# xiph/LPCNet

Hardware: AMD Instinct MI355X
Metric: 16 kHz samples/sec & concurrent real-time streams, 1/2/4/8 MI355X (higher is better)
Workload: dtype f32; 1 GPU; 2048 concurrent streams (each with its own feature file) per GPU x 25 frames (4000 samples) per step, fp32 weights, register-resident block-sparse GRU-A, bit-exact (PARITY) arithmetic; eight streams per CU as two groups of four half a step apart (BASELINE config 2's 1024 streams fill half of these stream slots: `also.config2_1024_streams`); arithmetic=parity, gru_a_blocks=1382, gru_a_densities=0.05,0.05,0.2 (benchmark model), gru_a_items_per_lane=30, streams_per_gpu=2048, streams_per_workgroup=8

## Files before the change

### lpcnet_amd/csrc/sample_kernel_x2.hip.h

```cpp
#pragma once
#include "sample_kernel.hip.h"
#include "tree_stages.h"

namespace lpcn {

#define LPCN_X2_LW 4
#define LPCN_X2_TW 0
#define LPCN_X2_S2W 7
#define LPCN_X2_S2_LEAD 2
#define LPCN_X2_HG 10

struct LdsX2 {
    static constexpr int S = 4;
    static constexpr int HA_STRIDE = 16 * S;
    static constexpr int g_hA    = 0;
    static constexpr int g_hT    = g_hA + 96 * HA_STRIDE + 24 * 16;
    static constexpr int g_prec  = g_hT + NA * S * 4;
    static constexpr int g_hB    = g_prec + NA * S * 4;
    static constexpr int g_idx   = g_hB + S * NB * 4;
    static constexpr int g_thr   = g_idx + S * 16;
    static constexpr int g_mask  = g_thr + S * 32;
    static constexpr int g_pfx   = g_mask + S * 4;
    static constexpr int g_lead  = g_mask + S * 64;
    static constexpr int g_flag  = g_lead + S * 32;
    static constexpr int g_condb = g_flag + 16;
    static constexpr int g_lpc   = g_condb + S * RB * 4;
    static constexpr int g_pcm   = g_lpc + S * 64;
    static constexpr int G_SZ    = g_pcm + S * 320;
    static constexpr int pre_ur  = 2 * G_SZ;
    static constexpr int inh     = pre_ur + 2 * NA * S * 4;
    static constexpr int abias   = inh + NA * S * 4;
    static constexpr int tansig  = abias + 2 * RA * 4;
    static constexpr int ulaw    = tansig + 816;
    static constexpr int logit   = ulaw + 1024;
    static constexpr int brec    = logit + 1024;
    static constexpr int bbias   = brec + NB * RB * 4;
    static constexpr int bstart  = bbias + 2 * RB * 4;
    static constexpr int bw      = bstart + 32;
    static constexpr int total(int nb_b) { return bw + (nb_b + 8) * 128; }
    __host__ __device__ static constexpr int ha_off(int p) { return p * HA_STRIDE + (p >> 2) * 16; }
};

typedef float tree_f4 __attribute__((ext_vector_type(4)));
struct TreeRow { tree_f4 w[NB / 4]; float bias, factor; };
__device__ __forceinline__ TreeRow tree_row_load_node(const LPCN_GLOBAL float *fc_w, const LPCN_GLOBAL float *fc_b, const LPCN_GLOBAL float *fc_f, const int node, const int chan)
{
    const auto *wp = (const LPCN_GLOBAL tree_f4 *)(fc_w + (node * 2 + chan) * NB);
    TreeRow r;
#pragma unroll
    for (int j = 0; j < NB / 4; ++j) r.w[j] = wp[j];
    r.bias = fc_b[chan * 256 + node];
    r.factor = fc_f[chan * 256 + node];
    return r;
}
template <int STAGE>
__device__ __forceinline__ TreeRow tree_row_load(const LPCN_GLOBAL float *fc_w, const LPCN_GLOBAL float *fc_b, const LPCN_GLOBAL float *fc_f, const int lane, const int prefix)
{
    return tree_row_load_node(fc_w, fc_b, fc_f, lpcn_tree_node(STAGE, lpcn_tree_lane_local(STAGE, lane), prefix), lane & 1);
}
__device__ __forceinline__ TreeRow tree_row_load_packed(const LPCN_GLOBAL float *fc_w, const LPCN_GLOBAL float *fc_b, const LPCN_GLOBAL float *fc_f, const int lane, const int prefix)
{
    return tree_row_load_node(fc_w, fc_b, fc_f, lpcn_tree_packed_node(lane, prefix), lane & 1);
}
__device__ __forceinline__ unsigned long long tree_node_ballot(const TreeRow &r, const float *h_s, const float *thr, const float *tansig)
{
    const float4 *hp = (const float4 *)h_s;
    float sum = r.bias;
#pragma unroll
    for (int j = 0; j < NB / 4; ++j) {
        const float4 hv = hp[j];
        const tree_f4 wv = r.w[j];
        sum = sum + wv[0] * hv.x;
        sum = sum + wv[1] * hv.y;
        sum = sum + wv[2] * hv.z;
        sum = sum + wv[3] * hv.w;
    }
    const float v = r.factor * lpcn_tanh(sum, tansig);
    const float vo = __builtin_bit_cast(float, __builtin_amdgcn_mov_dpp(__builtin_bit_cast(int, v), 0xB1, 0xf, 0xf, true));
    const float lg = v + vo;
    return __ballot(*thr < lg);
}
template <int STAGE>
__device__ __forceinline__ int tree_stage_walk(const TreeRow &r, const float *h_s, const float *thr_s, const float *tansig, const int lane)
{
    const unsigned long long m = tree_node_ballot(r, h_s, thr_s + lpcn_tree_level(STAGE, lpcn_tree_lane_local(STAGE, lane)), tansig) & lpcn_tree_stage_mask(STAGE);
    return lpcn_tree_stage_walk(m, STAGE == 0 ? LPCN_TREE_TOP : LPCN_TREE_LEVELS - LPCN_TREE_TOP);
}

template <int NW>
__global__ __launch_bounds__(LPCN_WG_THREADS, 2) void sample_kernel_x2(const LpcnSampleArgs *__restrict__ Ap)
{
    using L = LdsX2;
    constexpr int S = 4;
    constexpr int LW = LPCN_X2_LW, TW = LPCN_X2_TW;
    extern __shared__ __attribute__((aligned(16))) unsigned char smem[];
    float *const sm_pre_ur = (float *)(smem + L::pre_ur);
    float *const sm_inh = (float *)(smem + L::inh);
    const float *const sm_abias = (const float *)(smem + L::abias);
    const float *const sm_tansig = (const float *)(smem + L::tansig);
    const float *const sm_ulaw = (const float *)(smem + L::ulaw);
    const float *const sm_logit = (const float *)(smem + L::logit);
    const float *const sm_brec = (const float *)(smem + L::brec);
    const float *const sm_bbias = (const float *)(smem + L::bbias);
    const int *const sm_bstart = (const int *)(smem + L::bstart);

    const int tid0 = threadIdx.x;
    const int n_streams = Ap->n_streams, n_frames = Ap->n_frames, preload = Ap->preload, frame_len = Ap->frame_len;
    const int s0 = blockIdx.x * 2 * S;
    auto stream_of = [&](int gs) __attribute__((always_inline)) { return (s0 + gs < n_streams) ? s0 + gs : n_streams - 1; };
    const int n_valid = (n_streams - s0 < 2 * S) ? n_streams - s0 : 2 * S;
    const size_t nf = (size_t)n_frames;
    auto *const states = as_global_rw(Ap->state);
    const LPCN_GLOBAL float *emb_nat_sig = as_global(Ap->emb_nat_sig), *emb_nat_pred = as_global(Ap->emb_nat_pred), *emb_nat_exc = as_global(Ap->emb_nat_exc);
    asm volatile("" : "+s"(emb_nat_sig), "+s"(emb_nat_pred), "+s"(emb_nat_exc));

    float4 w[NW];
    uint32_t offp[(NW + 1) / 2];
    int row_reg[3];
#define LPCN_ROW(k) (row_reg[k])
    {
        const int lane = tid0 & 63, wave = tid0 >> 6;
        const size_t base = (size_t)wave * NW * 64 + lane;
        const int lane_sel = (lane & 3) * 16;
        const auto *ab = as_global(Ap->a_blk);
        const auto *aw = (const LPCN_GLOBAL float *)as_global(Ap->a_w);
#pragma unroll
        for (int j = 0; j < NW; ++j) {
            const auto *v = aw + (base + (size_t)j * 64) * 4;
            w[j] = make_float4(v[0], v[1], v[2], v[3]);
        }
#pragma unroll
        for (int j = 0; j < NW; j += 2) {
            const int p0 = ab[base + (size_t)j * 64];
            const int p1 = (j + 1 < NW) ? ab[base + (size_t)(j + 1) * 64] : 0;
            offp[j >> 1] = (uint32_t)(L::ha_off(p0) + lane_sel) | ((uint32_t)(L::ha_off(p1) + lane_sel) << 16);
        }
        const auto *ar = as_global(Ap->a_row);
#pragma unroll
        for (int k = 0; k < 3; ++k) row_reg[k] = ar[(wave * 3 + k) * 64 + lane];
    }
    int b1 = __builtin_amdgcn_readfirstlane(as_global(Ap->a_bound)[(tid0 >> 6) * 4 + 1]);
    int b2 = __builtin_amdgcn_readfirstlane(as_global(Ap->a_bound)[(tid0 >> 6) * 4 + 2]);
    int b3 = __builtin_amdgcn_readfirstlane(as_global(Ap->a_bound)[(tid0 >> 6) * 4 + 3]);
    const bool allh0 = __builtin_amdgcn_readfirstlane(as_global(Ap->a_allh)[(tid0 >> 6) * 3]) != 0;
    const LPCN_GLOBAL float *fc_w_s = as_global(Ap->fc_w), *fc_b_s = as_global(Ap->fc_b), *fc_f_s = as_global(Ap->fc_f);
    asm volatile("" : "+s"(fc_w_s), "+s"(fc_b_s), "+s"(fc_f_s));
    const LPCN_GLOBAL float *cond_a_s = as_global(Ap->cond_a);
    asm volatile("" : "+s"(cond_a_s));
    const int has_slot = __builtin_amdgcn_readfirstlane((__ballot(row_reg[0] >= 0) != 0ull ? 1 : 0) | (__ballot(row_reg[1] >= 0) != 0ull ? 2 : 0) |
                                                        (__ballot(row_reg[2] >= 0) != 0ull ? 4 : 0));
    const bool has2 = (has_slot & 4) != 0;
    const int hl = __builtin_amdgcn_readfirstlane(as_global(Ap->a_head)[tid0 >> 6]);
    const bool early_wave = hl > 0;
    const bool plain_start = __builtin_amdgcn_readfirstlane(((early_wave || __ballot(row_reg[0] >= 2 * NA) == 0ull) && __ballot(row_reg[1] >= 2 * NA || row_reg[2] >= 2 * NA) == 0ull) ? 1 : 0) != 0;

    {
        const int tid = tid0;
        stage_tables<L>(smem, Ap, tid, NB * RB);
        stage_grub_weights(smem + L::bw, Ap, tid, true);
        for (int i = tid; i < 2 * S * NA; i += LPCN_WG_THREADS) {
            const int gs = i / NA, n = i % NA, g = gs >> 2, s = gs & 3;
            const float hv0 = states[stream_of(gs)].gru_a[n];
            unsigned char *gb = smem + g * L::G_SZ;
            ((float *)(gb + L::g_hT))[n * S + s] = hv0;
            *(float *)(gb + L::g_hA + L::ha_off(n >> 2) + s * 16 + (n & 3) * 4) = hv0;
        }
        for (int i = tid; i < 2 * S * NB; i += LPCN_WG_THREADS) {
            const int gs = i / NB, g = gs >> 2, s = gs & 3;
            ((float *)(smem + g * L::G_SZ + L::g_hB))[s * NB + i % NB] = states[stream_of(gs)].gru_b[i % NB];
        }
        if (tid < 2 * S) {
            const int g = tid >> 2, s = tid & 3;
            unsigned char *gb = smem + g * L::G_SZ;
            stage_leader_record({(float *)(gb + L::g_lead), (int *)(gb + L::g_idx), nullptr, nullptr}, s, &states[stream_of(tid)]);
        }
        if (tid < 2) { int *fl = (int *)(smem + tid * L::G_SZ + L::g_flag); fl[0] = 0; fl[1] = 0; }
        if (tid < 2 * S) ((int *)(smem + (tid >> 2) * L::G_SZ + L::g_pfx))[tid & 3] = 0;
    }
    __syncthreads();

    const bool is_lw = (tid0 >> 6) == LW;
    const bool is_tw_lane = tid0 >= 64 * TW && tid0 < 64 * TW + S;
#define LPCN_LROW ((tid0 & 63) >> 4)
#define LPCN_TAP (tid0 & 15)
    float histP = is_lw ? states[stream_of(S + LPCN_LROW)].last_sig[LPCN_TAP] : 0.f;
    float histQ = is_lw ? states[stream_of(LPCN_LROW)].last_sig[LPCN_TAP] : 0.f;
    bool liveP = false, liveQ = false;
    int live_maskP = 0, live_maskQ = 0;
    int seqP = 0, seqQ = 0;
    int smpP = 0, smpQ = 0, fP = 0, fQ = 0;
    float lpc_tap = 0.f, prod_old = 0.f;

    const int T = n_frames * frame_len;
#if LPCN_ENABLE_PROF
#ifndef LPCN_PROF_MASK
#define LPCN_PROF_MASK 0xFFF
#endif
    unsigned long long *const prof = Ap->prof;
    unsigned long long pt[12] = {0, 0, 0, 0, 0, 0, 0, 0, 0, 0, 0, 0}, tprev = 0;
    const bool profiling = prof != nullptr && blockIdx.x == 0;
#define LPCN_X2_PROF(slot) do { if (((LPCN_PROF_MASK >> (slot)) & 1) && profiling) { const unsigned long long now_ = __builtin_amdgcn_s_memtime(); pt[slot] += now_ - tprev; tprev = now_; } } while (0)
    if (profiling) tprev = __builtin_amdgcn_s_memtime();
#else
#define LPCN_X2_PROF(slot) do { } while (0)
#endif
    for (int h = -1; h <= 2 * T + 1; ++h) {
        const int p = h & 1, q = p ^ 1;
        unsigned char *const gp = smem + p * L::G_SZ, *const gq = smem + q * L::G_SZ;
        const bool p_active = h >= 0 && (h >> 1) < T;
        const bool p_prev = h >= 2;
        const bool q_chain = h >= 1 && ((h - 1) >> 1) < T;
        const bool q_heads = ((h + 1) >> 1) < T;
        const bool new_frame = p_active && smpP == 0;
        const bool more = p_active && smpP != 0;
        float *const hT_p = (float *)(gp + L::g_hT);
        float *const hB_q = (float *)(gq + L::g_hB);
        int *const idx_p = (int *)(gp + L::g_idx);
        float *const lpc_p = (float *)(gp + L::g_lpc);
        short *const pcm_p = (short *)(gp + L::g_pcm);
        const LeaderCells cells_p = {(float *)(gp + L::g_lead), idx_p, (float *)(gp + L::g_thr), pcm_p};
        const uint32_t flag_p = lds_addr(gp + L::g_flag);

        if (more) ++seqP;
        if (p_prev && is_lw) {
            __builtin_amdgcn_s_setprio(3);
            const int smp_done = smpP == 0 ? frame_len - 1 : smpP - 1;
            int t_ = tid0;
            LPCN_REMAT_V(t_);
            const int lrow = (t_ & 63) >> 4, tap = t_ & 15;
            float pcm, deemph;
            int exc;
            draw_sample_walked(cells_p, (const int *)(gp + L::g_mask) + lrow, sm_ulaw, lrow, tap, liveP, smp_done, preload, histP, pcm, deemph, exc);
            if (more) { open_sample<S>(cells_p, tid0, liveP, pcm, tap == 0 ? pcm * lpc_tap : prod_old, exc, false); lds_publish(flag_p, seqP); }
            __builtin_amdgcn_s_setprio(0);
            finish_sample(cells_p, lrow, tap, liveP, smp_done, preload, pcm, deemph);
        }
        if (more && is_tw_lane && liveP) { int t_ = tid0; LPCN_REMAT_V(t_); draw_thresholds(cells_p, sm_logit, t_ - 64 * TW); }

        if (new_frame) {
            int tid = tid0;
            LPCN_REMAT_V(tid);
            const bool lw_ = (tid >> 6) == LW, twl_ = tid >= 64 * TW && tid < 64 * TW + S;
            __syncthreads();
            if (fP > 0) {
                auto *out = as_global_rw(Ap->pcm);
                const size_t pstride = (size_t)Ap->pcm_stride;
                for (int i = tid; i < S * LPCN_FRAME_SIZE; i += LPCN_WG_THREADS) {
                    const int s = i / LPCN_FRAME_SIZE, k = i % LPCN_FRAME_SIZE;
                    if (S * p + s < n_valid && k < frame_len) out[(size_t)(s0 + S * p + s) * pstride + (size_t)(fP - 1) * LPCN_FRAME_SIZE + k] = pcm_p[i];
                }
            }
            __syncthreads();
            {
                const auto *cb = as_global(Ap->cond_b), *lp = as_global(Ap->lpc);
                float *const condb_p = (float *)(gp + L::g_condb);
                if (tid < S * RB) condb_p[tid] = cb[((size_t)stream_of(S * p + tid / RB) * nf + fP) * RB + tid % RB];
                if (tid >= 256 && tid < 256 + S * LPCN_LPC_ORDER) {
                    const int i = tid - 256;
                    lpc_p[i] = lp[((size_t)stream_of(S * p + i / LPCN_LPC_ORDER) * nf + fP) * LPCN_LPC_ORDER + i % LPCN_LPC_ORDER];
                }
                if (lw_ || twl_) {
                    const int lstream = stream_of(S * p + (lw_ ? (tid & 63) >> 4 : tid - 64 * TW));
                    liveP = stream_is_live(Ap, states, lstream, fP);
                }
                if (preload > 0 && tid < S) {
                    const auto *pin = as_global(Ap->pcm) + (size_t)stream_of(S * p + tid) * (size_t)Ap->pcm_stride + (size_t)fP * LPCN_FRAME_SIZE;
                    for (int i = 0; i < preload; ++i) pcm_p[tid * LPCN_FRAME_SIZE + i] = pin[i];
                }
            }
            __syncthreads();
            ++seqP;
            if (lw_) {
                open_sample<S>(cells_p, tid0, liveP, histP, histP * lpc_p[tid & 63], ((const int *)cells_p.lead)[((tid & 63) >> 4) * 8 + 2], true);
                lds_publish(flag_p, seqP);
            }
            if (twl_ && liveP) draw_thresholds(cells_p, sm_logit, tid - 64 * TW);
            __syncthreads();
            int lm = 0;
#pragma unroll
            for (int s = 0; s < S; ++s) lm |= (idx_p[S + s] ? 1 : 0) << s;
            live_maskP = __builtin_amdgcn_readfirstlane(lm);
        }

        LPCN_X2_PROF(0);
        float acc[S] = {};
        constexpr int PF = 2;
        float4 hq[PF + 1] = {};
        const unsigned char *hA_cur = gp + L::g_hA;
        auto fetch_h = [&](const int j) __attribute__((always_inline)) {
            uint32_t pk = offp[j >> 1];
            LPCN_REMAT_V(pk);
            const uint32_t off = (j & 1) ? (pk >> 16) : (pk & 0xFFFFu);
            hq[j % (PF + 1)] = *(const float4 *)(hA_cur + off);
        };
        typedef float negz_t __attribute__((ext_vector_type(4)));
        negz_t negz = {-0.f, -0.f, -0.f, -0.f};
        auto load_negz = [&]() __attribute__((always_inline)) { negz = (negz_t){-0.f, -0.f, -0.f, -0.f}; asm volatile("" : "+v"(negz)); };
        auto mac = [&](const int j) __attribute__((always_inline)) {
            typedef float f4 __attribute__((ext_vector_type(4)));
            typedef float f2 __attribute__((ext_vector_type(2)));
            const float4 hv = hq[j % (PF + 1)];
            const float hk[4] = {hv.x, hv.y, hv.z, hv.w};
            const float wk[4] = {w[j].x, w[j].y, w[j].z, w[j].w};
            f2 a01 = {acc[0], acc[1]}, a23 = {acc[2], acc[3]};
            f4 pv[4];
#pragma unroll
            for (int c = 0; c < 4; ++c) pv[c] = __builtin_amdgcn_mfma_f32_4x4x1f32(hk[c], wk[c], negz, 0, 0, 0);
            __builtin_amdgcn_sched_barrier(0);
#pragma unroll
            for (int c = 0; c < 4; ++c) {
                a01 = a01 + __builtin_shufflevector(pv[c], pv[c], 0, 1);
                a23 = a23 + __builtin_shufflevector(pv[c], pv[c], 2, 3);
            }
            acc[0] = a01[0]; acc[1] = a01[1]; acc[2] = a23[0]; acc[3] = a23[1];
        };
        auto pre_cell = [&](const int r, unsigned char *gb) __attribute__((always_inline)) -> float * {
            return (float *)(r < 2 * NA ? smem + L::pre_ur + r * (S * 4) : gb + L::g_prec + (r - 2 * NA) * (S * 4));
        };

        const int wave = __builtin_amdgcn_readfirstlane(tid0 >> 6);

        constexpr int J0 = NW - LPCN_EARLY_MAX < 0 ? 0 : NW - LPCN_EARLY_MAX;
        constexpr int JM = J0 + LPCN_X2_HG < NW ? J0 + LPCN_X2_HG : NW;
        const bool do_heads = early_wave && q_heads;
        int e0 = NW - hl;
        LPCN_REMAT_S(e0);
        auto head_step = [&](auto self, auto jc, auto jend_c) __attribute__((always_inline)) -> void {
            constexpr int j = decltype(jc)::value, je = decltype(jend_c)::value;
            if constexpr (j < je) {
                if constexpr (j + PF < NW) fetch_h(j + PF);
                if (j >= e0) { asm volatile(""); mac(j); }
                self(self, std::integral_constant<int, j + 1>{}, jend_c);
            }
        };
        const uint32_t p0cnt_p = flag_p + 4;
        constexpr int CW = LPCN_X2_CHAIN_WAVES, P0W = LPCN_X2_P0_FIRST, NP0 = LPCN_WAVES - P0W;
        static_assert(NP0 * 64 * 3 == 2 * NA && CW == S, "three rounds of the row waves' lanes cover GRU-A's update / reset rows");
        const bool p0_wave = p_active && wave >= P0W;
        uint32_t o_sig[S] = {}, o_pred[S] = {}, o_exc[S] = {}, o_cond[S] = {};
        constexpr int P0PERM = 0x3102;
        int i0 = 0;
        float ld[3][4 * S] = {};
        auto p0_open = [&]() __attribute__((always_inline)) {
            int gi[S];
            {
                typedef int i4 __attribute__((ext_vector_type(4)));
                i4 v;
                int f;
                const uint32_t idx_a = lds_addr(idx_p);
                do {
                    asm volatile("ds_read_b32 %0, %2\n\tds_read_b128 %1, %3\n\ts_waitcnt lgkmcnt(0)" : "=&v"(f), "=&v"(v) : "v"(flag_p), "v"(idx_a) : "memory");
                    f = __builtin_amdgcn_readfirstlane(f);
                } while (f != seqP);
#pragma unroll
                for (int s = 0; s < S; ++s) gi[s] = __builtin_amdgcn_readfirstlane(v[s]);
            }
#pragma unroll
            for (int s = 0; s < S; ++s) {
                o_sig[s] = (uint32_t)(gi[s] & 0xFF) * (uint32_t)(RA * 4);
                o_pred[s] = (uint32_t)((gi[s] >> 8) & 0xFF) * (uint32_t)(RA * 4);
                o_exc[s] = ((uint32_t)(gi[s] >> 16) & 0xFFu) * (uint32_t)(RA * 4);
                o_cond[s] = (uint32_t)(((size_t)stream_of(S * p + s) * nf + (size_t)fP) * RA * 4);
            }
            int t_ = tid0;
            LPCN_REMAT_V(t_);
            i0 = (((P0PERM >> (4 * ((t_ >> 6) & 3))) & 3) << 6) | (t_ & 63);
        };
        const bool fifth = ((P0PERM >> (4 * (wave & 3))) & 3) < 2;
        auto issue = [&](const int k, const int buf) __attribute__((always_inline)) {
            const uint32_t rb = (uint32_t)(i0 + 256 * k) * 4u;
#pragma unroll
            for (int s = 0; s < S; ++s) {
                ld[buf][4 * s + 0] = *(const LPCN_GLOBAL float *)((const LPCN_GLOBAL char *)cond_a_s + (o_cond[s] + rb));
                ld[buf][4 * s + 1] = *(const LPCN_GLOBAL float *)((const LPCN_GLOBAL char *)emb_nat_sig + (o_sig[s] + rb));
                ld[buf][4 * s + 2] = *(const LPCN_GLOBAL float *)((const LPCN_GLOBAL char *)emb_nat_pred + (o_pred[s] + rb));
                ld[buf][4 * s + 3] = *(const LPCN_GLOBAL float *)((const LPCN_GLOBAL char *)emb_nat_exc + (o_exc[s] + rb));
            }
        };
        auto reduce = [&](const int k, const int buf) __attribute__((always_inline)) {
            const int r = i0 + 256 * k;
            float g[S];
#pragma unroll
            for (int s = 0; s < S; ++s) g[s] = ((ld[buf][4 * s + 0] + ld[buf][4 * s + 1]) + ld[buf][4 * s + 2]) + ld[buf][4 * s + 3];
            if (k < 3) {
                const int n = r >= NA ? r - NA : r;
                const float2 bd = *(const float2 *)(sm_abias + 2 * r);
                const float4 hv = *(const float4 *)(hT_p + n * S);
                *(float4 *)(sm_pre_ur + r * S) = make_float4((bd.x + bd.y * hv.x) + g[0], (bd.x + bd.y * hv.y) + g[1], (bd.x + bd.y * hv.z) + g[2], (bd.x + bd.y * hv.w) + g[3]);
            } else {
                *(float4 *)(sm_inh + (r - 2 * NA) * S) = make_float4(g[0], g[1], g[2], g[3]);
            }
        };
        if (wave < CW) {
            if (q_chain) {
                __builtin_amdgcn_s_setprio(3);
                const int s = wave;
                int ln_ = tid0;
                LPCN_REMAT_V(ln_);
                ln_ &= 63;
                const int r = ln_ < RB ? ln_ : RB - 1;
                const int g6 = r >> 3, ri = r & 7;
                const float *const condb_q = (const float *)(gq + L::g_condb);
                float zrh = sm_bbias[r] + condb_q[s * RB + r];
                float rec = sm_bbias[RB + r];
#pragma unroll
                for (int j = 0; j < NB; ++j) rec = rec + sm_brec[j * RB + r] * hB_q[s * NB + j];
                uint32_t wp32 = lds_addr(smem + L::bw + (sm_bstart[g6] * 8 + ri) * 16 + ((LPCN_GRUB_SHIFT >> (4 * g6)) & 15) * 128);
                uint32_t hp32 = lds_addr(gq + L::g_hA + s * 16);
                asm volatile(
#include "grub_lds_loop_s4.inc"
                    : [z] "+v"(zrh), [wp] "+v"(wp32), [hp] "+v"(hp32) : : LPCN_GRUB_LDS_CLOBBERS);
                __builtin_amdgcn_s_setprio(0);
                LPCN_X2_PROF(1);
                const TreeRow top = tree_row_load<0>(fc_w_s, fc_b_s, fc_f_s, ln_, 0);
                const int ln = ln_ & 15;
                const float sg = lpcn_sigmoid(zrh + rec, sm_tansig);
                const float r_gate = __builtin_bit_cast(float, __builtin_amdgcn_ds_bpermute((16 + ln) << 2, __builtin_bit_cast(int, sg)));
                const float hc = lpcn_tanh(zrh + rec * r_gate, sm_tansig);
                const float hc_i = __builtin_bit_cast(float, __builtin_amdgcn_ds_bpermute((32 + ln) << 2, __builtin_bit_cast(int, hc)));
                if (ln_ < NB) {
                    const float hold = hB_q[s * NB + ln_];
                    const float hnew = sg * hold + (1.f - sg) * hc_i;
                    if ((live_maskQ >> s) & 1) hB_q[s * NB + ln_] = hnew;
                }
                LPCN_X2_PROF(2);
                const float *const thr_s = (const float *)(gq + L::g_thr) + s * 8;
                const int val = tree_stage_walk<0>(top, hB_q + s * NB, thr_s, sm_tansig, ln_);
                if (ln_ == 0) lds_publish(lds_addr(gq + L::g_pfx) + s * 4, (seqQ << LPCN_TREE_TOP) | val);
                LPCN_X2_PROF(9);
            }
        } else {
            if (do_heads) {
                hA_cur = gq + L::g_hA;
                load_negz();
                {
                    int r = LPCN_ROW(0);
                    LPCN_REMAT_V(r);
                    r = r < 0 ? 0 : r;
                    const int n = r - 2 * NA;
                    const float bias = sm_abias[2 * r], diag = sm_abias[2 * r + 1];
                    const float *hT_q = (const float *)(gq + L::g_hT);
#pragma unroll
                    for (int s = 0; s < S; ++s) acc[s] = bias + diag * hT_q[n * S + s];
                }
#pragma unroll
                for (int j = 0; j < PF; ++j) if (J0 + j < NW) fetch_h(J0 + j);
                head_step(head_step, std::integral_constant<int, J0>{}, std::integral_constant<int, JM>{});
            }
            LPCN_X2_PROF(3);
            if (p0_wave) {
                p0_open();
                LPCN_X2_PROF(1);
                issue(0, 0); issue(1, 1); issue(2, 2);
                LPCN_X2_PROF(2);
                reduce(0, 0); reduce(1, 1); reduce(2, 2);
                lds_arrive(p0cnt_p);
                issue(3, 0);
                if (fifth) issue(4, 1);
            }
            LPCN_X2_PROF(4);
            if (do_heads) {
                head_step(head_step, std::integral_constant<int, JM>{}, std::integral_constant<int, NW>{});
                int r = LPCN_ROW(0);
                LPCN_REMAT_V(r);
                if (r >= 0) {
                    float *c = pre_cell(r, gq);
#pragma unroll
                    for (int s = 0; s < S; ++s) c[s] = acc[s];
                }
            }
            if (p0_wave) { reduce(3, 0); if (fifth) reduce(4, 1); }
            LPCN_X2_PROF(3);
        }

        static_assert(LPCN_X2_S2W > LPCN_X2_LW && LPCN_X2_S2W < LPCN_WAVES && LPCN_TREE_FIELDS == S && LPCN_X2_S2_LEAD >= 1, "stage 2 runs on a row wave other than the leader's, one field per stream");
        const bool s2_wave = q_chain && wave == LPCN_X2_S2W;
        TreeRow sub = {};
        int pfx = 0;
        auto s2_open = [&]() __attribute__((always_inline)) {
            int t_ = tid0;
            LPCN_REMAT_V(t_);
            const uint32_t cell = lds_addr(gq + L::g_pfx) + (uint32_t)lpcn_tree_packed_field(t_ & 63) * 4u;
            do {
                asm volatile("ds_read_b32 %0, %1\n\ts_waitcnt lgkmcnt(0)" : "=v"(pfx) : "v"(cell) : "memory");
            } while (__ballot((pfx >> LPCN_TREE_TOP) != seqQ) != 0ull);
            pfx &= (1 << LPCN_TREE_TOP) - 1;
            sub = tree_row_load_packed(fc_w_s, fc_b_s, fc_f_s, t_ & 63, pfx);
        };
        const bool s2_in_items = s2_wave && p_active && b3 > 0;
        if (s2_wave && !s2_in_items) s2_open();

        if (p_active) {
            hA_cur = gp + L::g_hA;
            load_negz();
            lds_poll_until<false>(p0cnt_p, seqP * NP0);
            LPCN_X2_PROF(11);
            if (plain_start) {
                int r = LPCN_ROW(0);
                LPCN_REMAT_V(r);
                r = r < 0 ? 0 : r;
                const float *c = pre_cell(r, gp);
#pragma unroll
                for (int s = 0; s < S; ++s) acc[s] = c[s];
            } else {
#pragma unroll
            for (int k = 0; k < 3; ++k) {
                int r = LPCN_ROW(k);
                LPCN_REMAT_V(r);
                const bool live_row = r >= 0;
                r = r < 0 ? 0 : r;
                const bool candidate = r >= 2 * NA;
                const int n = candidate ? r - 2 * NA : 0;
                const float bias = sm_abias[2 * r], diag = sm_abias[2 * r + 1];
                float *c = pre_cell(r, gp);
                const bool parked = k == 0 && early_wave;
#pragma unroll
                for (int s = 0; s < S; ++s) {
                    const float bv = bias + diag * hT_p[n * S + s];
                    if (k == 0) acc[s] = (candidate && !parked) ? bv : c[s];
                    else if (candidate && live_row) c[s] = bv;
                }
            }
            }
            auto row_swap = [&](const int k_done, const int k_next) __attribute__((always_inline)) {
                int r = LPCN_ROW(k_done), r2 = LPCN_ROW(k_next);
                LPCN_REMAT_V(r);
                LPCN_REMAT_V(r2);
                if (r >= 0) {
                    float *c = pre_cell(r, gp);
#pragma unroll
                    for (int s = 0; s < S; ++s) c[s] = acc[s];
                }
                r2 = r2 < 0 ? 0 : r2;
                const float *c2 = pre_cell(r2, gp);
#pragma unroll
                for (int s = 0; s < S; ++s) acc[s] = c2[s];
            };
            auto row_store = [&](const int k) __attribute__((always_inline)) {
                int r = LPCN_ROW(k);
                LPCN_REMAT_V(r);
                if (r >= 0) {
                    float *c = pre_cell(r, gp);
#pragma unroll
                    for (int s = 0; s < S; ++s) c[s] = acc[s];
                }
            };
            const int jend = b3;
            LPCN_X2_PROF(4);
#pragma unroll
            for (int j = 0; j < PF && j < NW; ++j) fetch_h(j);
            LPCN_REMAT_S(b1);
            LPCN_REMAT_S(b2);
            LPCN_REMAT_S(b3);
            int s2_at = s2_in_items ? (jend > LPCN_X2_S2_LEAD ? jend - LPCN_X2_S2_LEAD : 0) : NW + 1;
            LPCN_REMAT_S(s2_at);
            int nextb = b1 < s2_at ? b1 : s2_at;
            LPCN_REMAT_S(nextb);
            auto item = [&](const int j) __attribute__((always_inline)) -> bool {
                if (__builtin_expect(j >= jend, 0)) return false;
                if (j + PF < NW) fetch_h(j + PF);
                if (__builtin_expect(j == nextb, 0)) {
                    if (j == b1) row_swap(0, 1);
                    if (j == b2) row_swap(1, 2);
                    if (j == s2_at) s2_open();
                    __builtin_amdgcn_s_waitcnt(0xC07F);
                    nextb = b1 > j ? b1 : (b2 > j ? b2 : NW);
                    if (s2_at > j && s2_at < nextb) nextb = s2_at;
                }
                mac(j);
                return true;
            };
            auto run_items = [&](auto self, auto jc) __attribute__((always_inline)) -> void {
                constexpr int j = decltype(jc)::value;
                if constexpr (j < NW) {
                    if (!item(j)) return;
                    self(self, std::integral_constant<int, j + 1>{});
                }
            };
            run_items(run_items, std::integral_constant<int, 0>{});
            LPCN_X2_PROF(5);
            if (b1 >= jend) {
                row_swap(0, 1);
                row_swap(1, 2);
                row_store(2);
            } else if (b2 >= jend) {
                row_swap(1, 2);
                row_store(2);
            } else {
                row_store(2);
            }
            LPCN_X2_PROF(6);
        }
        if (s2_wave) {
            int t_ = tid0;
            LPCN_REMAT_V(t_);
            const int ln = t_ & 63, f = lpcn_tree_packed_field(ln);
            const unsigned long long m = tree_node_ballot(sub, hB_q + f * NB, (const float *)(gq + L::g_thr) + f * 8 + lpcn_tree_packed_level(ln), sm_tansig) & lpcn_tree_packed_mask();
            int walks = 0;
#pragma unroll
            for (int k = 0; k < S; ++k) walks |= lpcn_tree_packed_walk(m, k) << (8 * k);
            if ((ln & (LPCN_TREE_FIELD_LANES - 1)) == 0)
                ((int *)(gq + L::g_mask))[f] = (pfx << (LPCN_TREE_LEVELS - LPCN_TREE_TOP)) | ((walks >> (8 * f)) & ((1 << (LPCN_TREE_LEVELS - LPCN_TREE_TOP)) - 1));
        }
        if (q_chain && is_lw) {
            int t_ = tid0;
            LPCN_REMAT_V(t_);
            lpc_tap = ((const float *)(gq + L::g_lpc))[t_ & 63];
            prod_old = row_shr1(histQ, 0.f) * lpc_tap;
        }
        LPCN_X2_PROF(9);
        __syncthreads();
        LPCN_X2_PROF(7);

        int tid = tid0;
        LPCN_REMAT_V(tid);
        if (p_active) {
            constexpr int NI = NA * S, NQ = NI / LPCN_WG_THREADS;
            const float *const prec_p = (const float *)(gp + L::g_prec);
            float z[NQ], rg[NQ], a[NQ], hold[NQ];
#pragma unroll
            for (int k = 0; k < NQ; ++k) {
                const int i = tid + k * LPCN_WG_THREADS;
                z[k] = sm_pre_ur[i];
                rg[k] = sm_pre_ur[NI + i];
                a[k] = prec_p[i];
                hold[k] = hT_p[i];
            }
#pragma unroll
            for (int k = 0; k < NQ; ++k) { z[k] = lpcn_sigmoid(z[k], sm_tansig); rg[k] = lpcn_sigmoid(rg[k], sm_tansig); }
#pragma unroll
            for (int k = 0; k < NQ; ++k) a[k] = a[k] * rg[k] + sm_inh[tid + k * LPCN_WG_THREADS];
#pragma unroll
            for (int k = 0; k < NQ; ++k) a[k] = lpcn_tanh(a[k], sm_tansig);
            const unsigned ut = (unsigned)tid;
            const bool live_s = ((live_maskP >> (ut & 3u)) & 1) != 0;
            unsigned char *const ha0 = gp + L::g_hA + L::ha_off((int)(ut >> 4)) + (ut & 3u) * 16u + ((ut >> 2) & 3u) * 4u;
            static_assert(L::ha_off(32) == 32 * L::HA_STRIDE + 8 * 16 && LPCN_WG_THREADS == 512 && S == 4, "gate-stage address stride");
#pragma unroll
            for (int k = 0; k < NQ; ++k) {
                const float hnew = z[k] * hold[k] + (1.f - z[k]) * a[k];
                const float hv = live_s ? hnew : hold[k];
                hT_p[tid + k * LPCN_WG_THREADS] = hv;
                *(float *)(ha0 + k * L::ha_off(32)) = hv;
            }
        }
        LPCN_X2_PROF(8);
        __syncthreads();
        LPCN_X2_PROF(10);

        if (p_active) { if (++smpP == frame_len) { smpP = 0; ++fP; } }
        { const float t = histP; histP = histQ; histQ = t; }
        { const bool t = liveP; liveP = liveQ; liveQ = t; }
        { const int t = live_maskP; live_maskP = live_maskQ; live_maskQ = t; }
        { const int t = seqP; seqP = seqQ; seqQ = t; }
        { const int t = smpP; smpP = smpQ; smpQ = t; }
        { const int t = fP; fP = fQ; fQ = t; }
        asm volatile("; LPCN_SAMPLE_LOOP_END" ::: "memory");
        __builtin_amdgcn_sched_barrier(0);
    }

#if LPCN_ENABLE_PROF
    if (profiling && (tid0 & 63) == 0) {
#pragma unroll
        for (int i = 0; i < 12; ++i) prof[(tid0 >> 6) * 12 + i] += pt[i];
    }
#endif
    __syncthreads();
    {
        auto *out = as_global_rw(Ap->pcm);
        const size_t pstride = (size_t)Ap->pcm_stride;
        for (int i = tid0; i < 2 * S * LPCN_FRAME_SIZE; i += LPCN_WG_THREADS) {
            const int gs = i / LPCN_FRAME_SIZE, k = i % LPCN_FRAME_SIZE;
            const short *pb = (const short *)(smem + (gs >> 2) * L::G_SZ + L::g_pcm);
            if (gs < n_valid && k < frame_len) out[(size_t)(s0 + gs) * pstride + (size_t)(n_frames - 1) * LPCN_FRAME_SIZE + k] = pb[(gs & 3) * LPCN_FRAME_SIZE + k];
        }
    }
    {
        const int tid = tid0;
        for (int i = tid; i < 2 * S * NA; i += LPCN_WG_THREADS) {
            const int gs = i / NA, n = i % NA;
            if (gs < n_valid) states[s0 + gs].gru_a[n] = ((const float *)(smem + (gs >> 2) * L::G_SZ + L::g_hT))[n * S + (gs & 3)];
        }
        for (int i = tid; i < 2 * S * NB; i += LPCN_WG_THREADS) {
            const int gs = i / NB;
            if (gs < n_valid) states[s0 + gs].gru_b[i % NB] = ((const float *)(smem + (gs >> 2) * L::G_SZ + L::g_hB))[(gs & 3) * NB + i % NB];
        }
        if (is_lw) {
            if (LPCN_LROW < n_valid) states[s0 + LPCN_LROW].last_sig[LPCN_TAP] = histP;
            if (S + LPCN_LROW < n_valid) states[s0 + S + LPCN_LROW].last_sig[LPCN_TAP] = histQ;
        }
        if (tid < n_valid) {
            auto *st = &states[s0 + tid];
            const unsigned char *gb = smem + (tid >> 2) * L::G_SZ;
            const int *li = (const int *)(gb + L::g_lead) + (tid & 3) * 8;
            const float *lp = (const float *)(gb + L::g_lpc);
#pragma unroll
            for (int j = 0; j < LPCN_LPC_ORDER; ++j) st->lpc[j] = lp[(tid & 3) * LPCN_LPC_ORDER + j];
            st->deemph_mem = ((const float *)li)[1];
            st->last_exc = li[2];
#pragma unroll
            for (int j = 0; j < 4; ++j) st->rng[j] = (uint32_t)li[4 + j];
        }
    }
#undef LPCN_ROW
#undef LPCN_LROW
#undef LPCN_TAP
}

}
```

Baseline: 168.9 million samples/s.

## Precompute per-wave slot plan to skip empty row slots and move stage-2 wave

```diff
diff --git a/lpcnet_amd/csrc/sample_kernel_x2.hip.h b/lpcnet_amd/csrc/sample_kernel_x2.hip.h
--- a/lpcnet_amd/csrc/sample_kernel_x2.hip.h
+++ b/lpcnet_amd/csrc/sample_kernel_x2.hip.h
@@ -1,12 +1,13 @@
 #pragma once
 #include "sample_kernel.hip.h"
 #include "tree_stages.h"
+#include "slot_plan.h"
 
 namespace lpcn {
 
 #define LPCN_X2_LW 4
 #define LPCN_X2_TW 0
-#define LPCN_X2_S2W 7
+#define LPCN_X2_S2W 1
 #define LPCN_X2_S2_LEAD 2
 #define LPCN_X2_HG 10
 
@@ -152,7 +153,8 @@
     const bool has2 = (has_slot & 4) != 0;
     const int hl = __builtin_amdgcn_readfirstlane(as_global(Ap->a_head)[tid0 >> 6]);
     const bool early_wave = hl > 0;
-    const bool plain_start = __builtin_amdgcn_readfirstlane(((early_wave || __ballot(row_reg[0] >= 2 * NA) == 0ull) && __ballot(row_reg[1] >= 2 * NA || row_reg[2] >= 2 * NA) == 0ull) ? 1 : 0) != 0;
+    auto any_row = [&](const int k, const int lo, const int hi) __attribute__((always_inline)) { return __ballot(row_reg[k] >= lo && row_reg[k] < hi) != 0ull ? 1 << k : 0; };
+    int plan = __builtin_amdgcn_readfirstlane(lpcn_slot_plan(any_row(0, 0, RA) | any_row(1, 0, RA) | any_row(2, 0, RA), any_row(0, 2 * NA, RA) | any_row(1, 2 * NA, RA) | any_row(2, 2 * NA, RA), b1, b2, b3, hl));
 
     {
         const int tid = tid0;
@@ -473,7 +475,7 @@
             LPCN_X2_PROF(3);
         }
 
-        static_assert(LPCN_X2_S2W > LPCN_X2_LW && LPCN_X2_S2W < LPCN_WAVES && LPCN_TREE_FIELDS == S && LPCN_X2_S2_LEAD >= 1, "stage 2 runs on a row wave other than the leader's, one field per stream");
+        static_assert(LPCN_X2_S2W != LPCN_X2_LW && LPCN_X2_S2W >= 0 && LPCN_X2_S2W < LPCN_WAVES && LPCN_TREE_FIELDS == S && LPCN_X2_S2_LEAD >= 1, "stage 2 runs on any wave but the leader's, one field per stream");
         const bool s2_wave = q_chain && wave == LPCN_X2_S2W;
         TreeRow sub = {};
         int pfx = 0;
@@ -495,8 +497,11 @@
             load_negz();
             lds_poll_until<false>(p0cnt_p, seqP * NP0);
             LPCN_X2_PROF(11);
+            LPCN_REMAT_S(plan);
+            const bool plain_start = lpcn_slot_plain_start(plan);
+            const int first = lpcn_slot_first(plan);
             if (plain_start) {
-                int r = LPCN_ROW(0);
+                int r = first == 0 ? LPCN_ROW(0) : first == 1 ? LPCN_ROW(1) : LPCN_ROW(2);
                 LPCN_REMAT_V(r);
                 r = r < 0 ? 0 : r;
                 const float *c = pre_cell(r, gp);
@@ -505,6 +510,7 @@
             } else {
 #pragma unroll
             for (int k = 0; k < 3; ++k) {
+                if (k > 0 && !lpcn_slot_forms_start(plan, k)) continue;
                 int r = LPCN_ROW(k);
                 LPCN_REMAT_V(r);
                 const bool live_row = r >= 0;
@@ -513,7 +519,7 @@
                 const int n = candidate ? r - 2 * NA : 0;
                 const float bias = sm_abias[2 * r], diag = sm_abias[2 * r + 1];
                 float *c = pre_cell(r, gp);
-                const bool parked = k == 0 && early_wave;
+                const bool parked = lpcn_slot_parked(plan, k);
 #pragma unroll
                 for (int s = 0; s < S; ++s) {
                     const float bv = bias + diag * hT_p[n * S + s];
@@ -554,14 +560,15 @@
             LPCN_REMAT_S(b3);
             int s2_at = s2_in_items ? (jend > LPCN_X2_S2_LEAD ? jend - LPCN_X2_S2_LEAD : 0) : NW + 1;
             LPCN_REMAT_S(s2_at);
-            int nextb = b1 < s2_at ? b1 : s2_at;
+            int nextb = first >= 1 ? (first >= 2 || b2 <= 0 ? NW : b2) : b1;
+            if (s2_at < nextb) nextb = s2_at;
             LPCN_REMAT_S(nextb);
             auto item = [&](const int j) __attribute__((always_inline)) -> bool {
                 if (__builtin_expect(j >= jend, 0)) return false;
                 if (j + PF < NW) fetch_h(j + PF);
                 if (__builtin_expect(j == nextb, 0)) {
-                    if (j == b1) row_swap(0, 1);
-                    if (j == b2) row_swap(1, 2);
+                    if (lpcn_slot_moves(plan, 1, j, b1)) row_swap(0, 1);
+                    if (lpcn_slot_moves(plan, 2, j, b2)) row_swap(1, 2);
                     if (j == s2_at) s2_open();
                     __builtin_amdgcn_s_waitcnt(0xC07F);
                     nextb = b1 > j ? b1 : (b2 > j ? b2 : NW);
@@ -579,16 +586,9 @@
             };
             run_items(run_items, std::integral_constant<int, 0>{});
             LPCN_X2_PROF(5);
-            if (b1 >= jend) {
-                row_swap(0, 1);
-                row_swap(1, 2);
-                row_store(2);
-            } else if (b2 >= jend) {
-                row_swap(1, 2);
-                row_store(2);
-            } else {
-                row_store(2);
-            }
+            if (lpcn_slot_last(plan) == 0) row_store(0);
+            else if (lpcn_slot_last(plan) == 1) row_store(1);
+            else row_store(2);
             LPCN_X2_PROF(6);
         }
         if (s2_wave) {
diff --git a/lpcnet_amd/csrc/slot_plan.h b/lpcnet_amd/csrc/slot_plan.h
--- /dev/null
+++ b/lpcnet_amd/csrc/slot_plan.h
@@ -0,0 +1,18 @@
+#pragma once
+#include "lpcnet_math.h"
+
+LPCN_HD constexpr int lpcn_slot_plan(const int live, const int cand, const int b1, const int b2, const int b3, const int head)
+{
+    const int first = b3 <= 0 ? 0 : (b1 <= 0 ? 1 : 0) + (b2 <= 0 ? 1 : 0);
+    const int last = (b1 < b3 ? 1 : 0) + (b2 < b3 ? 1 : 0);
+    const int with_items = (b1 > 0 ? 1 : 0) + (b2 > b1 ? 1 : 0) + (b3 > b2 ? 1 : 0);
+    return (live & 7) | ((cand & 7) << 3) | ((head > 0 ? 1 : 0) << 6) | (first << 8) | (last << 10) | (with_items << 12);
+}
+LPCN_HD constexpr bool lpcn_slot_live(const int plan, const int k) { return ((plan >> k) & 1) != 0; }
+LPCN_HD constexpr bool lpcn_slot_parked(const int plan, const int k) { return k == 0 && ((plan >> 6) & 1) != 0; }
+LPCN_HD constexpr int lpcn_slot_with_items(const int plan) { return (plan >> 12) & 3; }
+LPCN_HD constexpr bool lpcn_slot_forms_start(const int plan, const int k) { return ((plan >> (3 + k)) & 1) != 0 && !lpcn_slot_parked(plan, k); }
+LPCN_HD constexpr bool lpcn_slot_plain_start(const int plan) { return !lpcn_slot_forms_start(plan, 0) && !lpcn_slot_forms_start(plan, 1) && !lpcn_slot_forms_start(plan, 2); }
+LPCN_HD constexpr int lpcn_slot_first(const int plan) { return lpcn_slot_plain_start(plan) ? (plan >> 8) & 3 : 0; }
+LPCN_HD constexpr int lpcn_slot_last(const int plan) { return (plan >> 10) & 3; }
+LPCN_HD constexpr bool lpcn_slot_moves(const int plan, const int k, const int j, const int b) { return j == b && (j > 0 || lpcn_slot_first(plan) < k); }
```

New measurement: 172.6 million samples/s (median of 6 runs). +2.2%, better.
